# zichunhao/lgn-autoencoder

Measured on AMD Instinct MI355X. Metric: jets/sec fwd+bwd, 30-particle maxdim=2 bs=512, higher is better.
Workload: dtype f64

## Files before the change

### include/lgn_amd.h

```cpp
#ifndef LGN_AMD_H
#define LGN_AMD_H

#include <stddef.h>
#include <stdint.h>

#ifdef __cplusplus
extern "C" {
#endif

#define LGN_AMD_ABI_VERSION 19

int lgn_abi_version(void);
const char* lgn_last_error(void);

int lgn_level_fwd_f64(int B, int N, int C, int CO, int decoder,
                      const double* s_in, const double* v_in, const double* p, const uint8_t* mask,
                      const double* ra, const double* rb, const double* rc,
                      const double* w0, const double* b0, const double* w1, const double* b1,
                      const double* wm0, const double* wm1,
                      double* ag0, double* ag1, double* s_out, double* v_out, void* stream);

int lgn_level_bwd_partial_rows(int B, int N, int decoder, int* rows_mix, int* rows_rad);
int lgn_level_rad_partial_len(int C, int decoder);
int lgn_level_jet_split(int B, int N);

int lgn_level_bwd_f64(int B, int N, int C, int CO, int decoder,
                      const double* s_in, const double* v_in, const double* p, const uint8_t* mask,
                      const double* ra, const double* rb, const double* rc,
                      const double* w0, const double* b0, const double* w1, const double* b1,
                      const double* wm0, const double* wm1, const double* ag0, const double* ag1,
                      const double* g_s_out, const double* g_v_out,
                      double* g_ag, double* g_s_in, double* g_v_in, double* g_p,
                      double* part_mix, double* part_rad, void* stream);

int lgn_cg_product_fwd_f64(int R, int N, int C, int D1, int D2, int DO, int mode, int nnz, const int* row_ptr, const int* col,
                           const double* coef, const double* x1, const double* x2, double* out, void* stream);
int lgn_cg_product_bwd_f64(int R, int N, int C, int D1, int D2, int DO, int mode, int nnz, const int* row_ptr, const int* col,
                           const double* coef, const double* x1, const double* x2, const double* g_out, double* g_x1, double* g_x2,
                           void* stream);

int lgn_reduce_partials_f64(const double* part, int rows, int n, double* out, int accumulate, void* stream);

int lgn_radial_finalize_f64(const double* tot, int C, const double* ra, const double* rb, const double* rc,
                            const double* w0, const double* w1,
                            double* g_a, double* g_b, double* g_c,
                            double* g_w0, double* g_b0, double* g_w1, double* g_b1, void* stream);

#define LGN_ACT_LEAKYRELU 0
#define LGN_ACT_RELU 1
#define LGN_ACT_ELU 2
#define LGN_ACT_SIGMOID 3
#define LGN_ACT_LOGSIGMOID 4
#define LGN_ACT_ATAN 5
#define LGN_ACT_COUNT 6
int lgn_cgmlp_fwd_f64(int M, int C, int H, int nlin, int activation, const double* const* w, const double* const* b,
                      const double* s_in, double* s_out, void* stream);
int lgn_cgmlp_partial_rows(int M, int H);
// ... 62 lines not shown
  int get_real;
  double jet_loss_scale;
} lgn_net_desc;
#define LGN_REAL_SUM 0
#define LGN_REAL_REAL 1
#define LGN_REAL_IMAG 2
#define LGN_REAL_MEAN 3
#define LGN_REAL_NORM 4
#define LGN_LOSS_CHAMFER 0
#define LGN_LOSS_MSE 1
#define LGN_LOSS_HUNGARIAN 2
typedef struct lgn_loss_desc {
  int kind;
  int abs_coord;
  int polar_coord;
  double scale;
} lgn_loss_desc;
#define LGN_POOL_MIN 0
#define LGN_POOL_MAX 1
#define LGN_POOL_MEAN 2
#define LGN_POOL_MIX 3
#define LGN_POOL(n, avg, o0, o1, o2, o3) ((n) | ((avg) << 3) | ((o0) << 4) | ((o1) << 6) | ((o2) << 8) | ((o3) << 10))
#define LGN_NET_NO_STATIC 1
#define LGN_NET_DEC_PAIRWISE 2
#define LGN_NET_LEVEL_V2 4
#define LGN_NET_MLP_V1 8
#define LGN_NET_MOMENTS_V1 16
#define LGN_NET_BWD_ORDERED 64
#define LGN_NET_DEC_UNFUSED 256
#define LGN_NET_MOMENTS_SPLIT 512
#define LGN_NET_MLP_BWD1 1024
#define LGN_NET_MLP_FULLTILE 2048
#define LGN_NET_LIVE_SCALARS 4096
#define LGN_NET_SPLIT_TAIL 128

#define LGN_LDS_LIMIT (160 * 1024)
long long lgn_encoder_end_lds_bytes(int N, int C0, int K, int CL, int Ts, int Tv, int pool);
long long lgn_decoder_end_lds_bytes(int N, int C0, int Tin, int CL);
long long lgn_junction_lds_bytes(int N, int CL, int Ts, int Tv, int pool, int C0);

int lgn_step_param_slots(const lgn_net_desc* d, int decoder);
long long lgn_step_workspace_doubles(const lgn_net_desc* d);
int lgn_step_fwd_bwd_f64(const lgn_net_desc* d, const double* params, double* grads, long long n_params,
                         const int64_t* enc_off, const int64_t* dec_off, const double* p4, const double* target,
                         const uint8_t* mask, const double* in_scalars, double* workspace, long long workspace_doubles,
                         double* recon, double* loss_part, const lgn_loss_desc* loss, int* assignment ,
                         int* status , void* stream);
#define LGN_FINALIZE_SCRATCH 2048
int lgn_step_finalize_f64(double* params, double* grads, long long n_params, const double* loss_part, int n_loss,
                          double l1_lambda, double* adam_m, double* adam_v, long long* step_dev,
                          double lr, double beta1, double beta2, double eps, int do_adam, double* loss_out, void* stream);
int lgn_step_train_f64(const lgn_net_desc* d, double* params, double* grads, long long n_params, const int64_t* enc_off,
                       const int64_t* dec_off, const double* p4, const double* target, const uint8_t* mask, const double* in_scalars,
                       double* workspace, long long workspace_doubles, double* recon, double* loss_part, int n_loss, double l1_lambda,
                       double* adam_m, double* adam_v, long long* step_dev, double lr, double beta1, double beta2, double eps,
                       int do_adam, double* loss_out, const lgn_loss_desc* loss, int* assignment ,
                       int* status , void* stream);

#define LGN_OPT_ADAM 0
#define LGN_OPT_RMSPROP 1
typedef struct {
  int kind;
  double l1_lambda, l2_lambda, lr, eps;
  double beta1, beta2;
  double alpha, momentum;
} lgn_optim_desc;
// ... 163 lines not shown
```

### lgn-autoencoder_amd/csrc/api.hip

```cpp
#include "net.hpp"

using namespace lgn;

extern "C" {

int lgn_level_fwd_f64(int B, int N, int C, int CO, int decoder, const double* s_in, const double* v_in, const double* p,
                      const uint8_t* mask, const double* ra, const double* rb, const double* rc, const double* w0,
                      const double* b0, const double* w1, const double* b1, const double* wm0, const double* wm1,
                      double* ag0, double* ag1, double* s_out, double* v_out, void* stream) {
  LGN_CHECK_ARG(s_in && v_in && p && b0 && b1 && wm0 && wm1 && ag0 && ag1 && s_out && v_out, "level_fwd: null pointer");
  LGN_CHECK_ARG(decoder || (mask && ra && rb && rc && w0 && w1), "level_fwd: encoder needs mask and radial parameters");
  LevelArgs<double> a{B, N, C, CO, s_in, v_in, p, mask, ra, rb, rc, w0, b0, w1, b1, wm0, wm1, ag0, ag1, s_out, v_out};
  a.flags = level_flags_from_env();
  return level_fwd_dispatch<double>(a, decoder, (hipStream_t)stream);
}

int lgn_level_bwd_partial_rows(int B, int N, int decoder, int* rows_mix, int* rows_rad) {
  LGN_CHECK_ARG(B > 0 && N > 0 && rows_mix && rows_rad, "level_bwd_partial_rows: bad arguments");
  level_bwd_partial_rows(B, N, decoder, level_flags_from_env(), rows_mix, rows_rad);
  return 0;
}

int lgn_level_rad_partial_len(int C, int decoder) { return rad_partial_size(C, decoder != 0); }
int lgn_level_jet_split(int B, int N) { return N <= 40 ? level_jet_split(B, N) : 1; }

int lgn_level_bwd_f64(int B, int N, int C, int CO, int decoder, const double* s_in, const double* v_in, const double* p,
                      const uint8_t* mask, const double* ra, const double* rb, const double* rc, const double* w0,
                      const double* b0, const double* w1, const double* b1, const double* wm0, const double* wm1,
                      const double* ag0, const double* ag1, const double* g_s_out, const double* g_v_out, double* g_ag,
                      double* g_s_in, double* g_v_in, double* g_p, double* part_mix, double* part_rad, void* stream) {
  LGN_CHECK_ARG(s_in && v_in && p && b0 && b1 && wm0 && wm1 && ag0 && ag1 && g_s_out && g_v_out && g_ag && g_s_in &&
                    g_v_in && part_mix && part_rad, "level_bwd: null pointer");
  LGN_CHECK_ARG(decoder ? (g_p != nullptr) : (mask && ra && rb && rc && w0 && w1), "level_bwd: missing decoder g_p / encoder radial parameters");
  LevelBwdArgs<double> a{B, N, C, CO, s_in, v_in, p, mask, ra, rb, rc, w0, b0, w1, b1, wm0, wm1, ag0, ag1,
                         g_s_out, g_v_out, g_ag, g_s_in, g_v_in, g_p, part_mix, part_rad};
  a.flags = level_flags_from_env();
  return level_bwd_dispatch<double>(a, decoder, (hipStream_t)stream);
}

int lgn_cg_product_fwd_f64(int R, int N, int C, int D1, int D2, int DO, int mode, int nnz, const int* row_ptr, const int* col,
                           const double* coef, const double* x1, const double* x2, double* out, void* stream) {
  return cg_product_fwd(R, N, C, D1, D2, DO, mode, nnz, row_ptr, col, coef, x1, x2, out, (hipStream_t)stream);
}
int lgn_cg_product_bwd_f64(int R, int N, int C, int D1, int D2, int DO, int mode, int nnz, const int* row_ptr, const int* col,
                           const double* coef, const double* x1, const double* x2, const double* g_out, double* g_x1, double* g_x2,
                           void* stream) {
  return cg_product_bwd(R, N, C, D1, D2, DO, mode, nnz, row_ptr, col, coef, x1, x2, g_out, g_x1, g_x2, (hipStream_t)stream);
}

int lgn_reduce_partials_f64(const double* part, int rows, int n, double* out, int accumulate, void* stream) {
  LGN_CHECK_ARG(part && out && rows > 0 && n >= 0, "reduce_partials: bad arguments");
  return reduce_partials<double>(part, rows, n, out, accumulate, (hipStream_t)stream);
}

int lgn_radial_finalize_f64(const double* tot, int C, const double* ra, const double* rb, const double* rc, const double* w0,
                            const double* w1, double* g_a, double* g_b, double* g_c, double* g_w0, double* g_b0,
                            double* g_w1, double* g_b1, void* stream) {
// ... 293 lines not shown
```

### lgn-autoencoder_amd/csrc/api_common.cpp

```cpp
#include <stdarg.h>
#include <stdlib.h>

#include "level.hpp"
#include "../../include/lgn_amd.h"

namespace lgn {
static thread_local char g_err[512] = "";
void set_error(const char* fmt, ...) {
  va_list ap;
  va_start(ap, fmt);
  vsnprintf(g_err, sizeof(g_err), fmt, ap);
  va_end(ap);
}
int level_flags_from_env() {
  auto on = [](const char* name) { const char* e = getenv(name); return e && e[0] == '1'; };
  return (on("LGN_AMD_DEC_PAIRWISE") ? LVL_DEC_PAIRWISE : 0) | (on("LGN_AMD_LEVEL_V2") ? LVL_LEVEL_V2 : 0) |
         (on("LGN_AMD_MOMENTS_V1") ? LVL_MOMENTS_V1 : 0) | (on("LGN_AMD_MLP_V1") ? LVL_MLP_V1 : 0) | (on("LGN_AMD_BWD_ORDERED") ? LVL_BWD_ORDERED : 0) |
         (on("LGN_AMD_MOMENTS_SPLIT") ? LVL_MOMENTS_SPLIT : 0) | (on("LGN_AMD_MLP_BWD1") ? LVL_MLP_BWD1 : 0) |
         (on("LGN_AMD_MLP_FULLTILE") ? LVL_MLP_FULLTILE : 0);
}
static_assert(LVL_DEC_PAIRWISE == LGN_NET_DEC_PAIRWISE && LVL_LEVEL_V2 == LGN_NET_LEVEL_V2 && LVL_MOMENTS_V1 == LGN_NET_MOMENTS_V1 &&
                  LVL_MLP_V1 == LGN_NET_MLP_V1 && LVL_MLP_BWD1 == LGN_NET_MLP_BWD1 && LVL_MLP_FULLTILE == LGN_NET_MLP_FULLTILE &&
                  LVL_BWD_ORDERED == LGN_NET_BWD_ORDERED && LVL_MOMENTS_SPLIT == LGN_NET_MOMENTS_SPLIT &&
                  LVL_LIVE_SCALARS == LGN_NET_LIVE_SCALARS, "LVL_* and LGN_NET_* are the same bits");
}

extern "C" {
const char* lgn_last_error(void) { return lgn::g_err; }
int lgn_abi_version(void) { return LGN_AMD_ABI_VERSION; }
}
```

### lgn-autoencoder_amd/csrc/level.hpp

```cpp
#pragma once
#include "common.hpp"

namespace lgn {

constexpr int LVL_DEC_PAIRWISE = 2;
constexpr int LVL_LEVEL_V2 = 4;
constexpr int LVL_MLP_V1 = 8;
constexpr int LVL_MOMENTS_V1 = 16;
constexpr int LVL_MLP_BWD1 = 1024;
constexpr int LVL_MLP_FULLTILE = 2048;
constexpr int LVL_MOMENTS_SPLIT = 512;
constexpr int LVL_LIVE_SCALARS = 4096;
constexpr int LVL_BWD_ORDERED = 64;
int level_flags_from_env();

template <typename T>
struct LevelArgs {
  int B, N, C, CO;
  const T* s_in;
  const T* v_in;
  const T* p;
  const uint8_t* mask;
  const T *ra, *rb, *rc, *w0, *b0, *w1, *b1;
  const T *wm0, *wm1;
  T* ag0;
  T* ag1;
  T* s_out;
  T* v_out;
  const T* in_w0 = nullptr;
  const T* in_w1 = nullptr;
  T* in_s = nullptr;
  T* in_v = nullptr;
  T* z1 = nullptr;
  size_t z1n = 0;
  T* z2 = nullptr;
  size_t z2n = 0;
  const T* loss_wo1 = nullptr;
  const T* loss_target = nullptr;
  T loss_scale = T(1);
  int loss_real = 0;
  T loss_jscale = T(0);
  T* loss_recon = nullptr;
  T* loss_part = nullptr;
  T* loss_gv = nullptr;
  T* loss_wpart = nullptr;
  int flags = 0;
// ... 4 lines not shown
struct LevelBwdArgs {
  int B, N, C, CO;
  const T *s_in, *v_in, *p;
  const uint8_t* mask;
  const T *ra, *rb, *rc, *w0, *b0, *w1, *b1;
  const T *wm0, *wm1;
  const T *ag0, *ag1;
  const T* g_s_out;
  const T* g_v_out;
  T* g_ag;
  T* g_s_in;
  T* g_v_in;
  T* g_p;
  T* part_mix;
  T* part_rad;
  T* part_in0 = nullptr;
  int flags = 0;
  int dead_scalars = 0;
};

__host__ __device__ constexpr int node_stride(int C) { return 10 * C + 4; }

__host__ __device__ constexpr int rad_partial_size(int C, bool dec) {
  return dec ? 2 * C : (2 * 4 * C * NB + 8 * C);
}

inline int level_jet_split(int B, int N) {
  const int groups = (N + 3) / 4;
  int s = 1;
  while (s * 2 <= groups && B * s * 2 <= 512) s *= 2;
  return s;
}

}
```

### lgn-autoencoder_amd/csrc/level_fwd2.hip

```cpp
#include "level_dev.hpp"
#include "net_dev.hpp"
#include "ops.hpp"
#include "wave_sum.hpp"

namespace lgn {

typedef double v4d __attribute__((ext_vector_type(4)));
LGN_STAMP_DECL
LGN_STAMP_READER(lgn_debug_stamps_fwd2)

__device__ __forceinline__ double dpp_quad(double v, int ctrl_is_xor2) {
  int lo = __double2loint(v), hi = __double2hiint(v);
  if (ctrl_is_xor2) {
    lo = __builtin_amdgcn_mov_dpp(lo, 0x4E, 0xF, 0xF, true);
    hi = __builtin_amdgcn_mov_dpp(hi, 0x4E, 0xF, 0xF, true);
  } else {
    lo = __builtin_amdgcn_mov_dpp(lo, 0xB1, 0xF, 0xF, true);
    hi = __builtin_amdgcn_mov_dpp(hi, 0xB1, 0xF, 0xF, true);
  }
  return __hiloint2double(hi, lo);
}
__device__ __forceinline__ double quad_sum(double v) {
  v += dpp_quad(v, 0);
  v += dpp_quad(v, 1);
  return v;
}

__device__ __forceinline__ double fast_rcp(double u) {
  double r = __builtin_amdgcn_rcp(u);
  double e = __builtin_fma(-u, r, 1.0);
  r = __builtin_fma(r, e, r);
  e = __builtin_fma(-u, r, 1.0);
  return __builtin_fma(r, e, r);
}

template <int C, bool DEC>
struct Fwd2 {
  static constexpr int NG = (C + 3) / 4;
  static constexpr int NS = node_stride(C);
  static constexpr int PS = DEC ? 8 : 4;
  static constexpr int AGS = 20 * C;
  static constexpr int A3 = 0, A4 = 2 * C, A1 = 4 * C, A2 = 12 * C;
};

template <int C, bool DEC, bool SEP, bool TRAIN, bool NOS>
__global__ __launch_bounds__(2 * BLOCK) void level_fwd2_kernel(LevelArgs<double> a, int chunk) {
  using F = Fwd2<C, DEC>;
  constexpr int NG = F::NG;
  const int N = a.N, B = a.B, CO = a.CO;
  const int b = blockIdx.x, tid = threadIdx.x, lane = tid & 63, wave = tid >> 6;
  const int nthr = blockDim.x, nw = nthr >> 6;

  extern __shared__ __align__(16) unsigned char smem_raw[];
  double* nd = reinterpret_cast<double*>(smem_raw);
  double* pj = nd + ((N * F::NS + 1) & ~1);
  double* wm = pj + N * F::PS;
  double* agl = wm + 4 * CO * 5 * C;
  double* sums = agl + chunk * F::AGS;
  uint8_t* mk = reinterpret_cast<uint8_t*>(sums + 20 * C);

  STAMP(0);
  if (!DEC && a.in_w0) {
    {
      const size_t wg = (size_t)blockIdx.y * gridDim.x + blockIdx.x, stride = (size_t)gridDim.x * gridDim.y * nthr;
      for (size_t e = wg * nthr + tid; e < a.z1n; e += stride) a.z1[e] = 0.0;
      for (size_t e = wg * nthr + tid; e < a.z2n; e += stride) a.z2[e] = 0.0;
    }
    const double* p0 = a.p + (size_t)b * N * 4;
    const size_t plane_s = (size_t)B * N * C;
    const int nw2 = 2 * CO * 5 * C;
    for (int e = tid; e < N * 4; e += nthr) pj[e] = p0[e];
    for (int e = tid; e < N; e += nthr) mk[e] = a.mask[(size_t)b * N + e];
    for (int e = tid; e < nw2; e += nthr) {
      wm[e] = a.wm0[e];
      wm[nw2 + e] = a.wm1[e];
    }
    for (int e = tid; e < N * C; e += nthr) {
      const int j = e / C, c = e - j * C;
      const double* p = p0 + j * 4;
      const double pe = p[0], px = p[1], py = p[2], pz = p[3];
      const double q0 = pe * pe, q1 = px * px, q2 = py * py, q3 = pz * pz;
      const double mass = sqrt(fabs(2.0 * q0 - (((q0 + q1) + q2) + q3)));
      constexpr double H = 0.70710678118654752440084436210484903928;
      const cx<double> q[4] = {{pe, 0.0}, {px * H, -py * H}, {pz, 0.0}, {-px * H, -py * H}};
      const double w0r = a.in_w0[c], w0i = a.in_w0[C + c];
      const cx<double> w1 = {a.in_w1[c], a.in_w1[C + c]};
      double* d = nd + j * F::NS + c * 10;
      d[0] = w0r * mass;
      d[1] = w0i * mass;
#pragma unroll
      for (int m = 0; m < 4; ++m) {
        const cx<double> r = cmul(w1, q[m]);
// ... 31 lines not shown
  const int ti = pr >> 2, tj = pr & 3;
  double ak[5], bk[5], ck2[5];
  double wf[NG][5];
  double bias[NG][4];
  if (!DEC) {
#pragma unroll
    for (int s = 0; s < 5; ++s) {
      const int k = 4 * s + cg;
      ak[s] = a.ra[k];
      bk[s] = a.rb[k];
      const double c = a.rc[k];
      ck2[s] = c * c;
    }
#pragma unroll
    for (int g = 0; g < NG; ++g) {
      const int rr = lane & 15, q = rr >> 2, ch = 4 * g + (rr & 3);
      const double* w = (q >> 1) ? a.w1 : a.w0;
#pragma unroll
      for (int s = 0; s < 5; ++s) wf[g][s] = ch < C ? w[(2 * ch + (q & 1)) * NB + 4 * s + cg] : 0.0;
    }
  }
#pragma unroll
  for (int g = 0; g < NG; ++g) {
    const int ch = 4 * g + cg;
#pragma unroll
    for (int q = 0; q < 4; ++q) {
      const double* bb = (q >> 1) ? a.b1 : a.b0;
      bias[g][q] = ch < C ? (DEC ? bb[ch] : bb[2 * ch + (q & 1)]) : 0.0;
    }
  }
  __syncthreads();
  STAMP(1);

  if constexpr (DEC && SEP) {
    if (tid < 64) {
      const int k = tid & 7, part = tid >> 3;
      double mean = 0.0;
      for (int n = part; n < N; n += 8) mean += pj[n * 8 + k];
      mean += shfl_xor(mean, 8);
      mean += shfl_xor(mean, 16);
      mean += shfl_xor(mean, 32);
      if (part == 0) sums[k] = mean / N;
    }
    __syncthreads();
    for (int e = tid; e < N * 8; e += nthr) pj[e] -= sums[e & 7];
    __syncthreads();
#define LGN_PUT(k, val)                                           \
  do {                                                            \
    if ((k) < 12) a0[(k) < 12 ? (k) : 0] += (val);                \
    else a1[(k) >= 12 ? (k) - 12 : 0] += (val);                   \
  } while (0)
    for (int c = wave; c < C; c += nw) {
      double a0[12], a1[8];
#pragma unroll
      for (int k = 0; k < 12; ++k) a0[k] = 0.0;
#pragma unroll
      for (int k = 0; k < 8; ++k) a1[k] = 0.0;
      for (int n = lane; n < N; n += 64) {
        const double* ni = nd + n * F::NS + c * 10;
        const double* pn = pj + n * 8;
        const cx<double> sn = {ni[0], ni[1]};
        cx<double> v[4], pc[4];
#pragma unroll
        for (int m = 0; m < 4; ++m) {
          v[m] = {ni[2 + m], ni[6 + m]};
          pc[m] = {pn[m], pn[4 + m]};
// ... 92 lines not shown
      const int rl = e / C, c = e - rl * C, n = c0 + rl;
      const double* sm = sums + c * 20;
      const double* pn = pj + n * 8;
      const cx<double> R0 = {a.b0[c], a.b0[c]}, R1 = {a.b1[c], a.b1[c]};
      const cx<double> e0 = {R0.r - R0.i, R0.r + R0.i};
      const cx<double> S = {sm[0], sm[1]};
      cx<double> VS[4], pc[4];
#pragma unroll
      for (int m = 0; m < 4; ++m) {
        VS[m] = {sm[2 + 2 * m], sm[3 + 2 * m]};
        pc[m] = {pn[m], pn[4 + m]};
      }
      double* st = agl + rl * F::AGS;
      if constexpr (!NOS) {
        const cx<double> a4 = cmul(S, e0);
        cx<double> t = bil2(VS, pc);
        t.r -= sm[18];  t.i -= sm[19];
        cx<double> a3 = cmul(R1, t);
        st[F::A3 + 2 * c] = 0.5 * a3.r;  st[F::A3 + 2 * c + 1] = 0.5 * a3.i;
        st[F::A4 + 2 * c] = a4.r;        st[F::A4 + 2 * c + 1] = a4.i;
      }
#pragma unroll
      for (int m = 0; m < 4; ++m) {
        const cx<double> a1 = cmul(VS[m], e0);
        cx<double> u = cmul(pc[m], S);
        u.r -= sm[10 + 2 * m];  u.i -= sm[11 + 2 * m];
        const cx<double> a2 = cmul(R1, u);
        st[F::A1 + (c * 4 + m) * 2] = a1.r;  st[F::A1 + (c * 4 + m) * 2 + 1] = a1.i;
        st[F::A2 + (c * 4 + m) * 2] = a2.r;  st[F::A2 + (c * 4 + m) * 2 + 1] = a2.i;
      }
    }
  } else {
  const int ngr = (c1 - c0 + 3) >> 2;
  const int rs = (!DEC && nw == 4 && ngr >= 1 && ngr <= 2 && chunk >= 16) ? 4 / ngr : 1;
  const int rpart = rs > 1 ? wave % rs : 0, ntl = (N + 3) >> 2;
  auto row_group = [&](const int rg, const int jlo, const int jhi, const int slab) __attribute__((always_inline)) {
    const int i0 = rg * 4;
    const int i = i0 + ti;
    const bool iok = i < N;
    const int ii = iok ? i : N - 1;
    double pi[F::PS];
#pragma unroll
    for (int m = 0; m < F::PS; ++m) pi[m] = pj[ii * F::PS + m];
    const bool mi = DEC ? false : (mk[ii] != 0);

    cx<double> A1[NG][4], A2[NG][4], A3[NG], A4[NG];
#pragma unroll
    for (int g = 0; g < NG; ++g) {
      A3[g] = {0, 0};
      A4[g] = {0, 0};
#pragma unroll
      for (int m = 0; m < 4; ++m) { A1[g][m] = {0, 0}; A2[g][m] = {0, 0}; }
    }

    STAMP(2 + ((rg >> 2) & 3) * 4);
    struct Tile {
      cx<double> q[4];
      double qd0, qd3, qa, qb;
      v4d R[NG];
      int jj;
      bool ok;
    };
    auto prep = [&](int j0, Tile& T) {
      const int j = j0 + tj;
      T.ok = iok && j < N;
      T.jj = j < N ? j : N - 1;
      const double* pjj = pj + T.jj * F::PS;
      if (DEC) {
#pragma unroll
        for (int m = 0; m < 4; ++m) T.q[m] = {pi[m] - pjj[m], pi[4 + m] - pjj[4 + m]};
#pragma unroll
        for (int g = 0; g < NG; ++g) T.R[g] = v4d{bias[g][0], bias[g][1], bias[g][2], bias[g][3]};
      } else {
        const double d0 = pi[0] - pjj[0], d1 = pi[1] - pjj[1], d2 = pi[2] - pjj[2], d3 = pi[3] - pjj[3];
        const double q0 = d0 * d0, q1 = d1 * d1, q2 = d2 * d2, q3 = d3 * d3;
        const double nsq = (2.0 * q0 - (((q0 + q1) + q2) + q3)) + 1e-16;
        const double an = fabs(nsq);
        const bool on = T.ok && mi && (mk[T.jj] != 0) && (nsq != 0.0);
        const double h = rsqrt2<double>();
        T.qd0 = d0;  T.qd3 = d3;  T.qa = d1 * h;  T.qb = d2 * h;
        double beta[5] = {0.0, 0.0, 0.0, 0.0, 0.0};
        if (on) {
#pragma unroll
          for (int s = 0; s < 5; ++s) beta[s] = 1.0 + ck2[s] * an;
          double rho5[5];
          rcp5(beta, rho5);
#pragma unroll
          for (int s = 0; s < 5; ++s) beta[s] = __builtin_fma(bk[s], rho5[s], ak[s]);
        }
#pragma unroll
        for (int g = 0; g < NG; ++g) {
          T.R[g] = v4d{bias[g][0], bias[g][1], bias[g][2], bias[g][3]};
#pragma unroll
          for (int s = 0; s < 5; ++s) T.R[g] = __builtin_amdgcn_mfma_f64_16x16x4f64(wf[g][s], beta[s], T.R[g], 0, 0, 0);
        }
      }
    };
    auto agg = [&](const Tile& T) {
      if (T.ok) {
        const double* nj = nd + T.jj * F::NS;
#pragma unroll
        for (int g = 0; g < NG; ++g) {
          const int ch = 4 * g + cg;
          if (ch < C) {
            const cx<double> R0 = {T.R[g][0], T.R[g][1]}, R1 = {T.R[g][2], T.R[g][3]};
            const cx<double> e0 = {R0.r - R0.i, R0.r + R0.i};
            const cx<double> sj = {nj[ch * 10], nj[ch * 10 + 1]};
            cx<double> vj[4];
#pragma unroll
            for (int m = 0; m < 4; ++m) {
              vj[m] = {nj[ch * 10 + 2 + m], nj[ch * 10 + 6 + m]};
// ... 31 lines not shown
          }
        }
      }
    };
    if (jlo < jhi) {
      Tile ta, tb;
      prep(jlo, ta);
      int j0 = jlo;
      while (true) {
        if (j0 + 4 < jhi) prep(j0 + 4, tb);
        agg(ta);
        j0 += 4;
        if (j0 >= jhi) break;
        if (j0 + 4 < jhi) prep(j0 + 4, ta);
        agg(tb);
        j0 += 4;
        if (j0 >= jhi) break;
      }
    }

    STAMP(3 + ((rg >> 2) & 3) * 4);
#pragma unroll
    for (int g = 0; g < NG; ++g) {
      if constexpr (!NOS) {
        A3[g].r = quad_sum(A3[g].r) * 0.5;  A3[g].i = quad_sum(A3[g].i) * 0.5;
        A4[g].r = quad_sum(A4[g].r);        A4[g].i = quad_sum(A4[g].i);
      }
#pragma unroll
      for (int m = 0; m < 4; ++m) {
        A1[g][m].r = quad_sum(A1[g][m].r);  A1[g][m].i = quad_sum(A1[g][m].i);
        A2[g][m].r = quad_sum(A2[g][m].r);  A2[g][m].i = quad_sum(A2[g][m].i);
      }
    }
    if (tj == 0) {
      double* st = agl + (slab + i0 + ti - c0) * F::AGS;
#pragma unroll
      for (int g = 0; g < NG; ++g) {
        const int ch = 4 * g + cg;
        if (ch < C) {
          if constexpr (!NOS) {
            st[F::A3 + 2 * ch] = A3[g].r;  st[F::A3 + 2 * ch + 1] = A3[g].i;
            st[F::A4 + 2 * ch] = A4[g].r;  st[F::A4 + 2 * ch + 1] = A4[g].i;
          }
#pragma unroll
          for (int m = 0; m < 4; ++m) {
            st[F::A1 + (ch * 4 + m) * 2] = A1[g][m].r;  st[F::A1 + (ch * 4 + m) * 2 + 1] = A1[g][m].i;
            st[F::A2 + (ch * 4 + m) * 2] = A2[g][m].r;  st[F::A2 + (ch * 4 + m) * 2 + 1] = A2[g][m].i;
          }
        }
      }
    }
    STAMP(4 + ((rg >> 2) & 3) * 4);
  };
  if (rs > 1) {
    const int rg = (c0 >> 2) + wave / rs;
    if (rg * 4 < c1) row_group(rg, 4 * (rpart * ntl / rs), min(N, 4 * ((rpart + 1) * ntl / rs)), rpart * 4 * ngr);
  } else {
    for (int rg = (c0 >> 2) + wave; rg * 4 < c1; rg += nw) row_group(rg, 0, N, 0);
  }
  if (rs > 1) {
    __syncthreads();
    const int tot = 4 * ngr * F::AGS;
    for (int e = tid; e < tot; e += nthr) {
      if (NOS && e % F::AGS < F::A1) continue;
      double v = agl[e];
      for (int pp = 1; pp < rs; ++pp) v += agl[pp * tot + e];
      agl[e] = v;
    }
  }
  }
  __syncthreads();
  STAMP(20);

  if constexpr (TRAIN) {
    const size_t pl0 = (size_t)B * N * 2 * C;
    if constexpr (!NOS) {
      for (int e = tid; e < (c1 - c0) * 2 * C; e += nthr) {
        const int n = e / (2 * C), r = e - n * 2 * C, blk = r / C, ch = r - blk * C;
        const double* st = agl + n * F::AGS + (blk ? F::A4 : F::A3) + 2 * ch;
        const size_t ge = ((size_t)b * N + c0) * 2 * C + e;
        a.ag0[ge] = st[0];
        a.ag0[pl0 + ge] = st[1];
      }
    }
    for (int e = tid; e < (c1 - c0) * 2 * C * 4; e += nthr) {
      const int n = e / (8 * C), r = e - n * 8 * C, blk = r / (4 * C), cm = r - blk * 4 * C;
      const double* st = agl + n * F::AGS + (blk ? F::A2 : F::A1) + 2 * cm;
      const size_t ge = ((size_t)b * N + c0) * 8 * C + e;
      a.ag1[ge] = st[0];
      a.ag1[pl0 * 4 + ge] = st[1];
    }
  }
  STAMP(21);

  catmix(c0, c1);
  STAMP(22);
  if (c1 < rhi) __syncthreads();
  }
  STAMP(40);
  if constexpr (DEC) {
    if (a.loss_wo1) {
      __syncthreads();
      dec_output_loss_body<TRAIN>(B, N, CO, a.v_out, a.loss_wo1, a.loss_target, a.loss_scale, a.loss_real, a.loss_jscale,
                                  a.loss_recon, a.loss_part, a.loss_gv, a.loss_wpart, smem_raw);
    }
  }
}

template <int C, bool DEC, bool SEP, bool TRAIN, bool NOS>
static int launch_level_fwd2(const LevelArgs<double>& a, hipStream_t stream) {
  using F = Fwd2<C, DEC>;
  const size_t fixed = sizeof(double) * (((size_t)a.N * F::NS + 1 & ~size_t(1)) + (size_t)a.N * F::PS + 4 * a.CO * 5 * C + 20 * C) + a.N + 16;
  const bool wide = a.B <= 320 && a.N >= 64;
  const size_t row = sizeof(double) * F::AGS, budget1 = 160 * 1024, budget2 = wide ? budget1 : 78 * 1024;
  const int full = (a.N + 15) & ~15;
  int chunk = full;
  if (fixed + full * row > budget2) {
    const size_t room = fixed + 16 * row <= budget2 ? budget2 - fixed : (fixed < budget1 ? budget1 - fixed : 0);
    chunk = (int)(room / row) & ~15;
    if (chunk > full) chunk = full;
    if (chunk < 16) chunk = 16;
  }
  size_t smem = fixed + chunk * row;
  if (a.loss_wo1) {
    LGN_CHECK_ARG(DEC && SEP && a.N <= 40 && !wide && a.loss_target && a.loss_recon && a.loss_part && (!TRAIN || (a.loss_gv && a.loss_wpart)),
                  "level_fwd: the loss rides on the separable decoder forward of jets of <= 40 particles only");
    if (smem < dec_out_loss_bytes(a.N, a.CO)) smem = dec_out_loss_bytes(a.N, a.CO);
  }
  LGN_CHECK_ARG(smem <= 160 * 1024, "level_fwd: N=%d C=%d needs %zu B of LDS (> 160 KiB)", a.N, a.C, smem);
  auto kern = level_fwd2_kernel<C, DEC, SEP, TRAIN, NOS>;
  if (smem > 64 * 1024) {
    hipError_t e = hipFuncSetAttribute(reinterpret_cast<const void*>(kern), hipFuncAttributeMaxDynamicSharedMemorySize, (int)smem);
    if (e != hipSuccess) { set_error("hipFuncSetAttribute: %s", hipGetErrorString(e)); return (int)e; }
  }
  const int nthreads = wide ? 2 * BLOCK : BLOCK;
  const int split = (SEP || a.N > 40) ? 1 : level_jet_split(a.B, a.N);
  hipLaunchKernelGGL(kern, dim3(a.B, split), dim3(nthreads), smem, stream, a, chunk);
  LGN_CHECK_LAUNCH();
  return 0;
}

bool level_fwd_carries_loss(int N, int flags) { return N <= 40 && !(flags & LVL_DEC_PAIRWISE); }

template <bool TRAIN, bool NOS>
static int level_fwd_run(const LevelArgs<double>& a, int decoder, hipStream_t stream) {
  LGN_CHECK_ARG(a.B > 0 && a.N > 0, "level_fwd: empty batch (B=%d N=%d)", a.B, a.N);
  LGN_CHECK_ARG(!a.in_w0 || (!decoder && a.in_w1 && a.in_s && a.in_v), "level_fwd: the input stage rides on encoder levels only");
  LGN_CHECK_ARG(a.CO >= 1 && a.CO <= 8, "level_fwd: C_out=%d unsupported (1..8)", a.CO);
  const bool pairwise = (a.flags & LVL_DEC_PAIRWISE) != 0;
#define LGN_CASE(CC)                                                                                         \
  case CC:                                                                                                   \
    if (!decoder) return launch_level_fwd2<CC, false, false, TRAIN, NOS>(a, stream);                         \
    return pairwise ? launch_level_fwd2<CC, true, false, TRAIN, NOS>(a, stream) : launch_level_fwd2<CC, true, true, TRAIN, NOS>(a, stream);
  switch (a.C) {
#ifdef LGN_DEV_ONLY_C4
    LGN_CASE(4)
#else
    LGN_CASE(1) LGN_CASE(2) LGN_CASE(3) LGN_CASE(4) LGN_CASE(5) LGN_CASE(6) LGN_CASE(7) LGN_CASE(8)
#endif
    default:
      set_error("level_fwd: C_in=%d unsupported (1..8)", a.C);
      return -1;
  }
#undef LGN_CASE
}

template <>
int level_fwd_dispatch<double>(const LevelArgs<double>& a, int decoder, hipStream_t stream) {
  return a.dead_scalars ? level_fwd_run<true, true>(a, decoder, stream) : level_fwd_run<true, false>(a, decoder, stream);
// ... 8 lines not shown
```

### lgn-autoencoder_amd/lgn/_native.py

```python
from __future__ import annotations

import ctypes as C
import os
from typing import Optional, Sequence

import torch

_HERE = os.path.dirname(os.path.abspath(__file__))
LIB_PATH = os.environ.get("LGN_AMD_LIB") or os.path.join(_HERE, "_lib", "liblgn_amd.so")
ABI_VERSION = 19
FINALIZE_SCRATCH = 2048
FINALIZE_OPT_SCRATCH = 4096

_lib: Optional[C.CDLL] = None

_vp, _i, _ip = C.c_void_p, C.c_int, C.POINTER(C.c_int)

_SIGNATURES = {
    "lgn_level_fwd_f64": [_i] * 5 + [_vp] * 18,
    "lgn_level_bwd_partial_rows": [_i, _i, _i, _ip, _ip],
    "lgn_level_rad_partial_len": [_i, _i],
    "lgn_level_jet_split": [_i, _i],
    "lgn_cg_product_fwd_f64": [_i] * 8 + [_vp] * 7,
    "lgn_cg_product_bwd_f64": [_i] * 8 + [_vp] * 9,
    "lgn_level_bwd_f64": [_i] * 5 + [_vp] * 24,
    "lgn_reduce_partials_f64": [_vp, _i, _i, _vp, _i, _vp],
    "lgn_radial_finalize_f64": [_vp, _i] + [_vp] * 13,
    "lgn_cgmlp_fwd_f64": [_i] * 5 + [_vp] * 5,
    "lgn_cgmlp_partial_rows": [_i, _i],
    "lgn_cgmlp_bwd_f64": [_i] * 5 + [_vp] * 6 + [_i, _vp],
    "lgn_mixreps_fwd_f64": [_i] * 4 + [_vp] * 4,
    "lgn_chamfer_f64": [_i] * 3 + [_vp] * 2 + [_i] + [_vp] * 4,
    "lgn_mixreps_partial_rows": [_i],
    "lgn_mixreps_bwd_f64": [_i] * 4 + [_vp] * 6,
}


class LocalTables(C.Structure):
    _fields_ = [("n_rows", C.c_int), ("n_out", C.c_int), ("n_w", C.c_int), ("n_terms", C.c_int), ("n_u", C.c_int),
                ("n_x", C.c_int), ("n_units", C.c_int), ("static_kind", C.c_int)] + [
        (name, C.c_void_p) for name in ("row_ptr", "t_type", "t_a", "t_b", "t_coef", "out_dim", "out_nblk", "out_row0", "out_q0",
                                        "out_w0", "u_ptr", "u_row", "u_coef", "x_ptr", "x_row", "x_other", "x_coef")] + [("h_out_w0", C.c_int * 8)]


_tp = C.POINTER(LocalTables)


_POOL_OPS = {"min": 0, "max": 1, "mean": 2, "average": 2}


def pool_code(map_to_latent: str):
    m = map_to_latent.lower()
    if m == "mix":
        return 1 | (3 << 4)
    if "&" in m and "+" in m:
# ... 21 lines not shown
        need = max(need, L.lgn_encoder_end_lds_bytes(n, ch[0], max(1, encoder.tau_input_scalars), ch[-1], ts, tv, code))
        if junction and decoder is not None:
            need = max(need, L.lgn_junction_lds_bytes(n, ch[-1], ts, tv, code, decoder.num_channels[0]))
    if decoder is not None:
        ch = decoder.num_channels
        need = max(need, L.lgn_decoder_end_lds_bytes(decoder.num_output_particles, ch[0], decoder.tau_latent_vectors, ch[-1]))
    return 0 <= need <= LDS_LIMIT


def pool_blocks(code: int) -> int:
    if code == 0:
        return 2
    return 1 if (code >> 3) & 1 else code & 7


class NetDesc(C.Structure):
    _fields_ = [("B", C.c_int), ("N", C.c_int), ("n_levels", C.c_int), ("enc_channels", C.c_int * 5),
                ("dec_channels", C.c_int * 5), ("tau_s", C.c_int), ("tau_v", C.c_int), ("mlp_hidden_mul", C.c_int),
                ("mlp_nlin", C.c_int), ("tau_v_in", C.c_int),
                ("enc_tables", _tp * 4), ("dec_tables", _tp * 4),
                ("enc_Q", C.c_int * 5), ("enc_qs", C.c_int * 5), ("enc_qv", C.c_int * 5),
                ("dec_Q", C.c_int * 5), ("dec_qs", C.c_int * 5), ("dec_qv", C.c_int * 5), ("flags", C.c_int),
                ("activation", C.c_int), ("n_in_scalars", C.c_int), ("latent_pool", C.c_int), ("dec_N", C.c_int),
                ("get_real", C.c_int), ("jet_loss_scale", C.c_double)]

    def __init__(self, *a, **kw):
        super().__init__(*a, **kw)
        self.flags = net_flags()


NET_NO_STATIC = 1
_NET_FLAG_ENV = {"LGN_AMD_NO_STATIC": 1, "LGN_AMD_DEC_PAIRWISE": 2, "LGN_AMD_LEVEL_V2": 4, "LGN_AMD_MLP_V1": 8,
                 "LGN_AMD_MOMENTS_V1": 16, "LGN_AMD_BWD_ORDERED": 64, "LGN_AMD_LIVE_SCALARS": 4096, "LGN_AMD_SPLIT_TAIL": 128, "LGN_AMD_DEC_UNFUSED": 256, "LGN_AMD_MOMENTS_SPLIT": 512,
                 "LGN_AMD_MLP_BWD1": 1024, "LGN_AMD_MLP_FULLTILE": 2048}
ACTIVATIONS = {"leakyrelu": 0, "relu": 1, "elu": 2, "sigmoid": 3, "logsigmoid": 4, "atan": 5}


def activation_id(name: str) -> int:
    try:
        return ACTIVATIONS[name.lower()]
    except KeyError:
        raise ValueError(f"Activation function {name} not implemented!") from None


def net_flags() -> int:
    return sum(bit for name, bit in _NET_FLAG_ENV.items() if os.environ.get(name, "") == "1")


class LossDesc(C.Structure):
    _fields_ = [("kind", C.c_int), ("abs_coord", C.c_int), ("polar_coord", C.c_int), ("scale", C.c_double)]


class OptimDesc(C.Structure):
    _fields_ = [("kind", C.c_int), ("l1_lambda", C.c_double), ("l2_lambda", C.c_double), ("lr", C.c_double), ("eps", C.c_double),
                ("beta1", C.c_double), ("beta2", C.c_double), ("alpha", C.c_double), ("momentum", C.c_double)]


OPT_ADAM, OPT_RMSPROP = 0, 1
LOSS_CHAMFER, LOSS_MSE, LOSS_HUNGARIAN = 0, 1, 2
ASSIGN_NMAX = 192
_dp = C.POINTER(NetDesc)
_lp = C.POINTER(LossDesc)
_op = C.POINTER(OptimDesc)
_ll = C.c_longlong
_d = C.c_double
_SIGNATURES.update({
    "lgn_moments_fwd_f64": [_i] * 5 + [_vp] * 12,
# ... 114 lines not shown
def ptr(t: Optional[torch.Tensor]):
    if t is None:
        return None
    if not t.is_cuda:
        raise RuntimeError("liblgn_amd.so operates on GPU tensors only (got a CPU tensor); there is no CPU fallback")
    if not t.is_contiguous():
        raise RuntimeError("non-contiguous tensor passed to the native library")
    return t.data_ptr()


def f64(t: torch.Tensor) -> torch.Tensor:
    if t.dtype != torch.float64:
        raise RuntimeError(f"the native path is fp64 (reference precision); got {t.dtype}")
    return t.contiguous()



def level_fwd(decoder, s_in, v_in, p, mask, rad, wm0, wm1):
    _, B, N, Cc = s_in.shape
    CO = wm0.shape[1]
    dev, dt = s_in.device, s_in.dtype
    ag0 = torch.empty(2, B, N, 2 * Cc, device=dev, dtype=dt)
    ag1 = torch.empty(2, B, N, 2 * Cc, 4, device=dev, dtype=dt)
    s_out = torch.empty(2, B, N, CO, device=dev, dtype=dt)
    v_out = torch.empty(2, B, N, CO, 4, device=dev, dtype=dt)
    a, b, c, w0, b0, w1, b1 = rad
    rc = lib().lgn_level_fwd_f64(B, N, Cc, CO, int(decoder), ptr(s_in), ptr(v_in), ptr(p), ptr(mask),
                                 ptr(a), ptr(b), ptr(c), ptr(w0), ptr(b0), ptr(w1), ptr(b1), ptr(wm0), ptr(wm1),
                                 ptr(ag0), ptr(ag1), ptr(s_out), ptr(v_out), stream_ptr())
    _check(rc, "lgn_level_fwd_f64")
    return ag0, ag1, s_out, v_out


def reduce_partials(part: torch.Tensor, out: torch.Tensor, accumulate: bool = False):
    rows, n = part.shape
    _check(lib().lgn_reduce_partials_f64(ptr(part), rows, n, ptr(out), int(accumulate), stream_ptr()),
           "lgn_reduce_partials_f64")
    return out


def level_bwd(decoder, s_in, v_in, p, mask, rad, wm0, wm1, ag0, ag1, g_s_out, g_v_out, g_p=None):
    _, B, N, Cc = s_in.shape
    CO = wm0.shape[1]
    dev, dt = s_in.device, s_in.dtype
    L = lib()
    rm, rr = C.c_int(), C.c_int()
    _check(L.lgn_level_bwd_partial_rows(B, N, int(decoder), C.byref(rm), C.byref(rr)), "lgn_level_bwd_partial_rows")
    nmix = 4 * CO * 5 * Cc
    nrad = L.lgn_level_rad_partial_len(Cc, int(decoder))
    part_mix = torch.empty(rm.value, nmix, device=dev, dtype=dt)
    part_rad = torch.empty(rr.value, nrad, device=dev, dtype=dt)
    g_ag = torch.empty(B, N, 20 * Cc, device=dev, dtype=dt)
    g_s_in = torch.empty_like(s_in)
    g_v_in = torch.empty_like(v_in)
    a, b, c, w0, b0, w1, b1 = rad
    rc = L.lgn_level_bwd_f64(B, N, Cc, CO, int(decoder), ptr(s_in), ptr(v_in), ptr(p), ptr(mask),
                             ptr(a), ptr(b), ptr(c), ptr(w0), ptr(b0), ptr(w1), ptr(b1), ptr(wm0), ptr(wm1),
                             ptr(ag0), ptr(ag1), ptr(g_s_out), ptr(g_v_out), ptr(g_ag), ptr(g_s_in), ptr(g_v_in),
                             ptr(g_p), ptr(part_mix), ptr(part_rad), stream_ptr())
    _check(rc, "lgn_level_bwd_f64")
    g_mix = torch.empty(nmix, device=dev, dtype=dt)
    reduce_partials(part_mix, g_mix)
    g_wm0 = g_mix[: nmix // 2].view(2, CO, 5 * Cc)
    g_wm1 = g_mix[nmix // 2:].view(2, CO, 5 * Cc)
    tot = torch.empty(nrad, device=dev, dtype=dt)
    reduce_partials(part_rad, tot)
# ... 174 lines not shown
```

Baseline: 1.109 million.

## Compact encoder pairwise sweep to real particles and add closed-form padding contributions

```diff
diff --git a/include/lgn_amd.h b/include/lgn_amd.h
--- a/include/lgn_amd.h
+++ b/include/lgn_amd.h
@@ -23,6 +23,9 @@
 int lgn_level_bwd_partial_rows(int B, int N, int decoder, int* rows_mix, int* rows_rad);
 int lgn_level_rad_partial_len(int C, int decoder);
 int lgn_level_jet_split(int B, int N);
+
+int lgn_jet_order_host(const int* counts, int B, int ncu, int* order);
+int lgn_jet_order_mask(const uint8_t* mask, int B, int N, int ncu, int* order, void* stream);
 
 int lgn_level_bwd_f64(int B, int N, int C, int CO, int decoder,
                       const double* s_in, const double* v_in, const double* p, const uint8_t* mask,
@@ -151,6 +154,7 @@
 #define LGN_NET_MLP_BWD1 1024
 #define LGN_NET_MLP_FULLTILE 2048
 #define LGN_NET_LIVE_SCALARS 4096
+#define LGN_NET_ENC_FULL_SWEEP 8192
 #define LGN_NET_SPLIT_TAIL 128
 
 #define LGN_LDS_LIMIT (160 * 1024)
diff --git a/lgn-autoencoder_amd/csrc/api.hip b/lgn-autoencoder_amd/csrc/api.hip
--- a/lgn-autoencoder_amd/csrc/api.hip
+++ b/lgn-autoencoder_amd/csrc/api.hip
@@ -23,6 +23,24 @@
 
 int lgn_level_rad_partial_len(int C, int decoder) { return rad_partial_size(C, decoder != 0); }
 int lgn_level_jet_split(int B, int N) { return N <= 40 ? level_jet_split(B, N) : 1; }
+
+int lgn_jet_order_host(const int* counts, int B, int ncu, int* order) {
+  LGN_CHECK_ARG(counts && order && B > 0 && ncu > 0, "jet_order_host: bad arguments");
+  for (int b = 0; b < B; ++b) {
+    LGN_CHECK_ARG(counts[b] >= 0, "jet_order_host: counts[%d] = %d < 0", b, counts[b]);
+    int D = 0, E = 0, k = 0;
+    for (int o = 0; o < B; ++o) {
+      D += counts[o] > counts[b];
+      E += counts[o] == counts[b];
+      k += counts[o] == counts[b] && o < b;
+    }
+    order[jet_order_slot(D, E, k, B, ncu)] = b;
+  }
+  return 0;
+}
+int lgn_jet_order_mask(const uint8_t* mask, int B, int N, int ncu, int* order, void* stream) {
+  return jet_order_launch(mask, B, N, ncu, order, (hipStream_t)stream);
+}
 
 int lgn_level_bwd_f64(int B, int N, int C, int CO, int decoder, const double* s_in, const double* v_in, const double* p,
                       const uint8_t* mask, const double* ra, const double* rb, const double* rc, const double* w0,
diff --git a/lgn-autoencoder_amd/csrc/api_common.cpp b/lgn-autoencoder_amd/csrc/api_common.cpp
--- a/lgn-autoencoder_amd/csrc/api_common.cpp
+++ b/lgn-autoencoder_amd/csrc/api_common.cpp
@@ -17,12 +17,13 @@
   return (on("LGN_AMD_DEC_PAIRWISE") ? LVL_DEC_PAIRWISE : 0) | (on("LGN_AMD_LEVEL_V2") ? LVL_LEVEL_V2 : 0) |
          (on("LGN_AMD_MOMENTS_V1") ? LVL_MOMENTS_V1 : 0) | (on("LGN_AMD_MLP_V1") ? LVL_MLP_V1 : 0) | (on("LGN_AMD_BWD_ORDERED") ? LVL_BWD_ORDERED : 0) |
          (on("LGN_AMD_MOMENTS_SPLIT") ? LVL_MOMENTS_SPLIT : 0) | (on("LGN_AMD_MLP_BWD1") ? LVL_MLP_BWD1 : 0) |
-         (on("LGN_AMD_MLP_FULLTILE") ? LVL_MLP_FULLTILE : 0);
+         (on("LGN_AMD_MLP_FULLTILE") ? LVL_MLP_FULLTILE : 0) | (on("LGN_AMD_ENC_FULL_SWEEP") ? LVL_ENC_FULL_SWEEP : 0);
 }
 static_assert(LVL_DEC_PAIRWISE == LGN_NET_DEC_PAIRWISE && LVL_LEVEL_V2 == LGN_NET_LEVEL_V2 && LVL_MOMENTS_V1 == LGN_NET_MOMENTS_V1 &&
                   LVL_MLP_V1 == LGN_NET_MLP_V1 && LVL_MLP_BWD1 == LGN_NET_MLP_BWD1 && LVL_MLP_FULLTILE == LGN_NET_MLP_FULLTILE &&
                   LVL_BWD_ORDERED == LGN_NET_BWD_ORDERED && LVL_MOMENTS_SPLIT == LGN_NET_MOMENTS_SPLIT &&
-                  LVL_LIVE_SCALARS == LGN_NET_LIVE_SCALARS, "LVL_* and LGN_NET_* are the same bits");
+                  LVL_LIVE_SCALARS == LGN_NET_LIVE_SCALARS && LVL_ENC_FULL_SWEEP == LGN_NET_ENC_FULL_SWEEP,
+              "LVL_* and LGN_NET_* are the same bits");
 }
 
 extern "C" {
diff --git a/lgn-autoencoder_amd/csrc/level.hpp b/lgn-autoencoder_amd/csrc/level.hpp
--- a/lgn-autoencoder_amd/csrc/level.hpp
+++ b/lgn-autoencoder_amd/csrc/level.hpp
@@ -12,6 +12,7 @@
 constexpr int LVL_MOMENTS_SPLIT = 512;
 constexpr int LVL_LIVE_SCALARS = 4096;
 constexpr int LVL_BWD_ORDERED = 64;
+constexpr int LVL_ENC_FULL_SWEEP = 8192;
 int level_flags_from_env();
 
 template <typename T>
@@ -82,4 +83,13 @@
   return s;
 }
 
+__host__ __device__ inline int jet_order_slot(int D, int E, int k, int B, int ncu) {
+  const int r = D + k;
+  if (B <= ncu || B > 2 * ncu || r < ncu) return r;
+  const int kcut = ncu > D ? ncu - D : 0;
+  return ncu + (B - D - E) + (k - kcut);
 }
+constexpr int JET_ORDER_MAX_B = 8192;
+int jet_order_launch(const uint8_t* mask, int B, int N, int ncu, int* order, hipStream_t stream);
+
+}
diff --git a/lgn-autoencoder_amd/csrc/level_fwd2.hip b/lgn-autoencoder_amd/csrc/level_fwd2.hip
--- a/lgn-autoencoder_amd/csrc/level_fwd2.hip
+++ b/lgn-autoencoder_amd/csrc/level_fwd2.hip
@@ -41,12 +41,14 @@
   static constexpr int PS = DEC ? 8 : 4;
   static constexpr int AGS = 20 * C;
   static constexpr int A3 = 0, A4 = 2 * C, A1 = 4 * C, A2 = 12 * C;
+  static constexpr int NSUM = (DEC ? 20 : 40) * C;
 };
 
-template <int C, bool DEC, bool SEP, bool TRAIN, bool NOS>
+template <int C, bool DEC, bool SEP, bool TRAIN, bool NOS, bool CMP>
 __global__ __launch_bounds__(2 * BLOCK) void level_fwd2_kernel(LevelArgs<double> a, int chunk) {
   using F = Fwd2<C, DEC>;
   constexpr int NG = F::NG;
+  static_assert(!CMP || (!DEC && !SEP), "the compacted sweep is the encoder's");
   const int N = a.N, B = a.B, CO = a.CO;
   const int b = blockIdx.x, tid = threadIdx.x, lane = tid & 63, wave = tid >> 6;
   const int nthr = blockDim.x, nw = nthr >> 6;
@@ -57,7 +59,8 @@
   double* wm = pj + N * F::PS;
   double* agl = wm + 4 * CO * 5 * C;
   double* sums = agl + chunk * F::AGS;
-  uint8_t* mk = reinterpret_cast<uint8_t*>(sums + 20 * C);
+  uint8_t* mk = reinterpret_cast<uint8_t*>(sums + F::NSUM);
+  uint8_t* ridx = mk + N;
 
   STAMP(0);
   if (!DEC && a.in_w0) {
@@ -155,6 +158,64 @@
   __syncthreads();
   STAMP(1);
 
+  int nreal = N;
+  double pmean[4] = {0.0, 0.0, 0.0, 0.0};
+  if constexpr (CMP) {
+    const bool real = lane < N && mk[lane < N ? lane : 0] != 0;
+    const unsigned long long bal = __ballot(real);
+    nreal = __popcll(bal);
+    if (wave == 0 && real) ridx[__popcll(bal & ((1ull << lane) - 1ull))] = (uint8_t)lane;
+    if (nreal < N) {
+      {
+        double m8[8], s8[8];
+#pragma unroll
+        for (int k = 0; k < 4; ++k) { m8[k] = lane < N ? pj[(lane < N ? lane : 0) * 4 + k] : 0.0; m8[4 + k] = 0.0; }
+        wave_allsum<8>(m8, s8, lane);
+#pragma unroll
+        for (int k = 0; k < 4; ++k) pmean[k] = s8[k] / N;
+      }
+      for (int c = wave; c < C; c += nw) {
+        double t[20];
+#pragma unroll
+        for (int k = 0; k < 20; ++k) t[k] = 0.0;
+        if (lane < N) {
+          const double* ni = nd + lane * F::NS + c * 10;
+          const double* pn = pj + lane * 4;
+          const double h = rsqrt2<double>();
+          const double d0 = pn[0] - pmean[0], qa = (pn[1] - pmean[1]) * h, qb = (pn[2] - pmean[2]) * h, d3 = pn[3] - pmean[3];
+          const cx<double> pc[4] = {{d0, 0.0}, {qa, -qb}, {d3, 0.0}, {-qa, -qb}};
+          const cx<double> sn = {ni[0], ni[1]};
+          cx<double> v[4];
+#pragma unroll
+          for (int m = 0; m < 4; ++m) v[m] = {ni[2 + m], ni[6 + m]};
+          t[0] = sn.r;  t[1] = sn.i;
+#pragma unroll
+          for (int m = 0; m < 4; ++m) {
+            t[2 + 2 * m] = v[m].r;  t[3 + 2 * m] = v[m].i;
+            const cx<double> sp = cmul(sn, pc[m]);
+            t[10 + 2 * m] = sp.r;  t[11 + 2 * m] = sp.i;
+          }
+          if constexpr (!NOS) {
+            const cx<double> vp = bil2(v, pc);
+            t[18] = vp.r;  t[19] = vp.i;
+          }
+        }
+#pragma unroll
+        for (int set = 0; set < 2; ++set) {
+          const bool in = lane < N && (real == (set == 0));
+          double a0[12], a1[8];
+#pragma unroll
+          for (int k = 0; k < 12; ++k) a0[k] = in ? t[k] : 0.0;
+#pragma unroll
+          for (int k = 0; k < 8; ++k) a1[k] = in ? t[12 + k] : 0.0;
+          wave_sum_store<12>(a0, sums + set * 20 * C + c * 20, lane);
+          wave_sum_store<8>(a1, sums + set * 20 * C + c * 20 + 12, lane);
+        }
+      }
+    }
+    __syncthreads();
+  }
+
   if constexpr (DEC && SEP) {
     if (tid < 64) {
       const int k = tid & 7, part = tid >> 3;
@@ -313,17 +374,18 @@
     }
   } else {
   const int ngr = (c1 - c0 + 3) >> 2;
-  const int rs = (!DEC && nw == 4 && ngr >= 1 && ngr <= 2 && chunk >= 16) ? 4 / ngr : 1;
+  const int rs = (!DEC && !CMP && nw == 4 && ngr >= 1 && ngr <= 2 && chunk >= 16) ? 4 / ngr : 1;
   const int rpart = rs > 1 ? wave % rs : 0, ntl = (N + 3) >> 2;
+  const int NN = CMP ? nreal : N;
   auto row_group = [&](const int rg, const int jlo, const int jhi, const int slab) __attribute__((always_inline)) {
     const int i0 = rg * 4;
     const int i = i0 + ti;
-    const bool iok = i < N;
-    const int ii = iok ? i : N - 1;
+    const bool iok = i < NN;
+    const int ii = CMP ? ridx[iok ? i : NN - 1] : (iok ? i : N - 1);
     double pi[F::PS];
 #pragma unroll
     for (int m = 0; m < F::PS; ++m) pi[m] = pj[ii * F::PS + m];
-    const bool mi = DEC ? false : (mk[ii] != 0);
+    const bool mi = DEC ? false : (CMP || mk[ii] != 0);
 
     cx<double> A1[NG][4], A2[NG][4], A3[NG], A4[NG];
 #pragma unroll
@@ -344,8 +406,8 @@
     };
     auto prep = [&](int j0, Tile& T) {
       const int j = j0 + tj;
-      T.ok = iok && j < N;
-      T.jj = j < N ? j : N - 1;
+      T.ok = iok && j < NN;
+      T.jj = CMP ? ridx[j < NN ? j : NN - 1] : (j < N ? j : N - 1);
       const double* pjj = pj + T.jj * F::PS;
       if (DEC) {
 #pragma unroll
@@ -357,7 +419,7 @@
         const double q0 = d0 * d0, q1 = d1 * d1, q2 = d2 * d2, q3 = d3 * d3;
         const double nsq = (2.0 * q0 - (((q0 + q1) + q2) + q3)) + 1e-16;
         const double an = fabs(nsq);
-        const bool on = T.ok && mi && (mk[T.jj] != 0) && (nsq != 0.0);
+        const bool on = T.ok && mi && (CMP || mk[T.jj] != 0) && (nsq != 0.0);
         const double h = rsqrt2<double>();
         T.qd0 = d0;  T.qd3 = d3;  T.qa = d1 * h;  T.qb = d2 * h;
         double beta[5] = {0.0, 0.0, 0.0, 0.0, 0.0};
@@ -455,8 +517,8 @@
         A2[g][m].r = quad_sum(A2[g][m].r);  A2[g][m].i = quad_sum(A2[g][m].i);
       }
     }
-    if (tj == 0) {
-      double* st = agl + (slab + i0 + ti - c0) * F::AGS;
+    if (tj == 0 && (!CMP || iok)) {
+      double* st = agl + (CMP ? ii : slab + i0 + ti - c0) * F::AGS;
 #pragma unroll
       for (int g = 0; g < NG; ++g) {
         const int ch = 4 * g + cg;
@@ -479,7 +541,7 @@
     const int rg = (c0 >> 2) + wave / rs;
     if (rg * 4 < c1) row_group(rg, 4 * (rpart * ntl / rs), min(N, 4 * ((rpart + 1) * ntl / rs)), rpart * 4 * ngr);
   } else {
-    for (int rg = (c0 >> 2) + wave; rg * 4 < c1; rg += nw) row_group(rg, 0, N, 0);
+    for (int rg = (c0 >> 2) + wave; rg * 4 < (CMP ? NN : c1); rg += nw) row_group(rg, 0, NN, 0);
   }
   if (rs > 1) {
     __syncthreads();
@@ -493,6 +555,53 @@
   }
   }
   __syncthreads();
+  if constexpr (CMP) {
+    if (nreal < N) {
+      for (int e = tid; e < N * C; e += nthr) {
+        const int n = e / C, c = e - n * C;
+        const bool real = mk[n] != 0;
+        const double* sr = sums + c * 20;
+        const double* sp = sums + 20 * C + c * 20;
+        double sm[20];
+#pragma unroll
+        for (int k = 0; k < 20; ++k) sm[k] = real ? sp[k] : sr[k] + sp[k];
+        const double* pn = pj + n * 4;
+        const double h = rsqrt2<double>();
+        const double d0 = pn[0] - pmean[0], qa = (pn[1] - pmean[1]) * h, qb = (pn[2] - pmean[2]) * h, d3 = pn[3] - pmean[3];
+        const cx<double> pc[4] = {{d0, 0.0}, {qa, -qb}, {d3, 0.0}, {-qa, -qb}};
+        const cx<double> R0 = {a.b0[2 * c], a.b0[2 * c + 1]}, R1 = {a.b1[2 * c], a.b1[2 * c + 1]};
+        const cx<double> e0 = {R0.r - R0.i, R0.r + R0.i};
+        const cx<double> S = {sm[0], sm[1]};
+        cx<double> VS[4];
+#pragma unroll
+        for (int m = 0; m < 4; ++m) VS[m] = {sm[2 + 2 * m], sm[3 + 2 * m]};
+        double* st = agl + n * F::AGS;
+        auto put = [&](double* dst, cx<double> val) {
+          dst[0] = real ? dst[0] + val.r : val.r;
+          dst[1] = real ? dst[1] + val.i : val.i;
+        };
+        if constexpr (!NOS) {
+          const cx<double> a4 = cmul(S, e0);
+          cx<double> t = bil2(VS, pc);
+          t.r -= sm[18];  t.i -= sm[19];
+          cx<double> a3 = cmul(R1, t);
+          a3.r *= 0.5;  a3.i *= 0.5;
+          put(st + F::A3 + 2 * c, a3);
+          put(st + F::A4 + 2 * c, a4);
+        }
+#pragma unroll
+        for (int m = 0; m < 4; ++m) {
+          const cx<double> a1 = cmul(VS[m], e0);
+          cx<double> u = cmul(pc[m], S);
+          u.r -= sm[10 + 2 * m];  u.i -= sm[11 + 2 * m];
+          const cx<double> a2 = cmul(R1, u);
+          put(st + F::A1 + (c * 4 + m) * 2, a1);
+          put(st + F::A2 + (c * 4 + m) * 2, a2);
+        }
+      }
+      __syncthreads();
+    }
+  }
   STAMP(20);
 
   if constexpr (TRAIN) {
@@ -530,10 +639,57 @@
   }
 }
 
+__global__ __launch_bounds__(1024) void jet_order_kernel(const uint8_t* __restrict__ mask, int B, int N, int ncu, int* __restrict__ order) {
+  __shared__ unsigned short kidx[JET_ORDER_MAX_B];
+  __shared__ uint8_t cnt[JET_ORDER_MAX_B];
+  __shared__ int tot[64], above[64];
+  const int tid = threadIdx.x, lane = tid & 63, wave = tid >> 6, nw = blockDim.x >> 6;
+  for (int b = tid; b < B; b += blockDim.x) {
+    const uint8_t* m = mask + (size_t)b * N;
+    int n = 0;
+    for (int j = 0; j < N; ++j) n += m[j] != 0;
+    cnt[b] = (uint8_t)n;
+  }
+  __syncthreads();
+  for (int c = wave; c <= N; c += nw) {
+    int base = 0;
+    for (int b0 = 0; b0 < B; b0 += 64) {
+      const int b = b0 + lane;
+      const bool hit = b < B && cnt[b] == c;
+      const unsigned long long bal = __ballot(hit);
+      if (hit) kidx[b] = (unsigned short)(base + __popcll(bal & ((1ull << lane) - 1ull)));
+      base += __popcll(bal);
+    }
+    if (lane == 0) tot[c] = base;
+  }
+  __syncthreads();
+  if (tid == 0) {
+    int run = 0;
+    for (int c = N; c >= 0; --c) { above[c] = run; run += tot[c]; }
+  }
+  __syncthreads();
+  for (int b = tid; b < B; b += blockDim.x) {
+    const int c = cnt[b];
+    order[jet_order_slot(above[c], tot[c], kidx[b], B, ncu)] = b;
+  }
+}
+
+int jet_order_launch(const uint8_t* mask, int B, int N, int ncu, int* order, hipStream_t stream) {
+  LGN_CHECK_ARG(mask && order && B > 0 && B <= JET_ORDER_MAX_B && N > 0 && N < 64 && ncu > 0, "jet_order: B=%d N=%d unsupported", B, N);
+  hipLaunchKernelGGL(jet_order_kernel, dim3(1), dim3(1024), 0, stream, mask, B, N, ncu, order);
+  LGN_CHECK_LAUNCH();
+  return 0;
+}
+
+template <int C>
+static bool fwd2_compacts(const LevelArgs<double>& a, int chunk, int split) {
+  return !(a.flags & LVL_ENC_FULL_SWEEP) && a.N <= 40 && split == 1 && chunk >= a.N;
+}
+
 template <int C, bool DEC, bool SEP, bool TRAIN, bool NOS>
 static int launch_level_fwd2(const LevelArgs<double>& a, hipStream_t stream) {
   using F = Fwd2<C, DEC>;
-  const size_t fixed = sizeof(double) * (((size_t)a.N * F::NS + 1 & ~size_t(1)) + (size_t)a.N * F::PS + 4 * a.CO * 5 * C + 20 * C) + a.N + 16;
+  const size_t fixed = sizeof(double) * (((size_t)a.N * F::NS + 1 & ~size_t(1)) + (size_t)a.N * F::PS + 4 * a.CO * 5 * C + F::NSUM) + 2 * a.N + 16;
   const bool wide = a.B <= 320 && a.N >= 64;
   const size_t row = sizeof(double) * F::AGS, budget1 = 160 * 1024, budget2 = wide ? budget1 : 78 * 1024;
   const int full = (a.N + 15) & ~15;
@@ -551,13 +707,16 @@
     if (smem < dec_out_loss_bytes(a.N, a.CO)) smem = dec_out_loss_bytes(a.N, a.CO);
   }
   LGN_CHECK_ARG(smem <= 160 * 1024, "level_fwd: N=%d C=%d needs %zu B of LDS (> 160 KiB)", a.N, a.C, smem);
-  auto kern = level_fwd2_kernel<C, DEC, SEP, TRAIN, NOS>;
+  const int split = (SEP || a.N > 40) ? 1 : level_jet_split(a.B, a.N);
+  auto kern = level_fwd2_kernel<C, DEC, SEP, TRAIN, NOS, false>;
+  if constexpr (!DEC && !SEP) {
+    if (fwd2_compacts<C>(a, chunk, split)) kern = level_fwd2_kernel<C, DEC, SEP, TRAIN, NOS, true>;
+  }
   if (smem > 64 * 1024) {
     hipError_t e = hipFuncSetAttribute(reinterpret_cast<const void*>(kern), hipFuncAttributeMaxDynamicSharedMemorySize, (int)smem);
     if (e != hipSuccess) { set_error("hipFuncSetAttribute: %s", hipGetErrorString(e)); return (int)e; }
   }
   const int nthreads = wide ? 2 * BLOCK : BLOCK;
-  const int split = (SEP || a.N > 40) ? 1 : level_jet_split(a.B, a.N);
   hipLaunchKernelGGL(kern, dim3(a.B, split), dim3(nthreads), smem, stream, a, chunk);
   LGN_CHECK_LAUNCH();
   return 0;
diff --git a/lgn-autoencoder_amd/lgn/_native.py b/lgn-autoencoder_amd/lgn/_native.py
--- a/lgn-autoencoder_amd/lgn/_native.py
+++ b/lgn-autoencoder_amd/lgn/_native.py
@@ -21,6 +21,8 @@
     "lgn_level_bwd_partial_rows": [_i, _i, _i, _ip, _ip],
     "lgn_level_rad_partial_len": [_i, _i],
     "lgn_level_jet_split": [_i, _i],
+    "lgn_jet_order_host": [_ip, _i, _i, _ip],
+    "lgn_jet_order_mask": [_vp, _i, _i, _i, _vp, _vp],
     "lgn_cg_product_fwd_f64": [_i] * 8 + [_vp] * 7,
     "lgn_cg_product_bwd_f64": [_i] * 8 + [_vp] * 9,
     "lgn_level_bwd_f64": [_i] * 5 + [_vp] * 24,
@@ -108,7 +110,7 @@
 NET_NO_STATIC = 1
 _NET_FLAG_ENV = {"LGN_AMD_NO_STATIC": 1, "LGN_AMD_DEC_PAIRWISE": 2, "LGN_AMD_LEVEL_V2": 4, "LGN_AMD_MLP_V1": 8,
                  "LGN_AMD_MOMENTS_V1": 16, "LGN_AMD_BWD_ORDERED": 64, "LGN_AMD_LIVE_SCALARS": 4096, "LGN_AMD_SPLIT_TAIL": 128, "LGN_AMD_DEC_UNFUSED": 256, "LGN_AMD_MOMENTS_SPLIT": 512,
-                 "LGN_AMD_MLP_BWD1": 1024, "LGN_AMD_MLP_FULLTILE": 2048}
+                 "LGN_AMD_MLP_BWD1": 1024, "LGN_AMD_MLP_FULLTILE": 2048, "LGN_AMD_ENC_FULL_SWEEP": 8192}
 ACTIVATIONS = {"leakyrelu": 0, "relu": 1, "elu": 2, "sigmoid": 3, "logsigmoid": 4, "atan": 5}
 
 
@@ -289,6 +291,21 @@
     return ag0, ag1, s_out, v_out
 
 
+def jet_order_host(counts, ncu: int):
+    counts = [int(c) for c in counts]
+    B = len(counts)
+    cin, out = (C.c_int * B)(*counts), (C.c_int * B)()
+    _check(lib().lgn_jet_order_host(cin, B, int(ncu), out), "lgn_jet_order_host")
+    return list(out)
+
+
+def jet_order_mask(mask: torch.Tensor, ncu: int) -> torch.Tensor:
+    B, N = mask.shape
+    order = torch.empty(B, device=mask.device, dtype=torch.int32)
+    _check(lib().lgn_jet_order_mask(ptr(mask), B, N, int(ncu), ptr(order), stream_ptr()), "lgn_jet_order_mask")
+    return order
+
+
 def reduce_partials(part: torch.Tensor, out: torch.Tensor, accumulate: bool = False):
     rows, n = part.shape
     _check(lib().lgn_reduce_partials_f64(ptr(part), rows, n, ptr(out), int(accumulate), stream_ptr()),
```

Result: slower. 1.089 million (-1.8%).
